# b4rtaz/distributed-llama

Measured on AMD Instinct MI355X. Metric: decode tokens/s (Llama-3.1-8B Q40), higher is better.
Workload: dtype f32-accum/int8-dot (Q40 weights, Q80 activations); 1 GPU; model=llama-3.1-8b, global_batch=1, seq_len=4096, prefill=32, parallelism=tp1, sync=q80, graph=True

## Files before the change

dllama_amd/ops/csrc/gemv.hip:

```cpp

#include "dllama_common.h"

__device__ __forceinline__ int q40_block_dot(const uint4 wq, const int4 x0,
                                             const int4 x1) {
    const uint32_t wv[4] = {wq.x, wq.y, wq.z, wq.w};
    const int32_t xv[8] = {x0.x, x0.y, x0.z, x0.w, x1.x, x1.y, x1.z, x1.w};
    int idot = 0;
    #pragma unroll
    for (int wi = 0; wi < 4; wi++) {
        idot = dot4((int)(wv[wi] & 0x0F0F0F0Fu), xv[wi], idot);
        idot = dot4((int)((wv[wi] >> 4) & 0x0F0F0F0Fu), xv[4 + wi], idot);
    }
    return idot;
}

#define EPI_NONE 0
#define EPI_PACK 4
#define EPI_RESID_Q 3
#define EPI_RESID 1
#define EPI_ROPE 2

template <int NB, int RPW, int EPI, int PRO>
__global__ void k_q40_gemv(const uint8_t *__restrict__ qs,
                           const __half *__restrict__ scales,
                           const int8_t *__restrict__ xq,
                           const float *__restrict__ xs,
                           const float *__restrict__ xbs,
                           float *__restrict__ y,
                           int d, int n,
                           unsigned long long *__restrict__ amax_scratch,
                           float *__restrict__ x_resid,
                           float *__restrict__ ssq,
                           const float *__restrict__ rope_cache,
                           const int *__restrict__ pos,
                           float *__restrict__ kc,
                           float *__restrict__ vc,
                           int q_dim0, int kv_dim0, int hd,
                           const float *__restrict__ wnorm,
                           const float *__restrict__ ssq_in,
                           float eps, int kv_f16,
                           int8_t *__restrict__ oqq,
                           float *__restrict__ oqs,
                           float *__restrict__ oqbs) {
    const int wpb = blockDim.x / WAVE;
    const int wid = threadIdx.x / WAVE;
    const int row0 = (blockIdx.x * wpb + wid) * RPW;
    const int lane = threadIdx.x % WAVE;
    const int nb = n / QB;
    const int nbp = nb >> 1;
    const int nks = gridDim.y;
    const int j0p = (int)((int64_t)nbp * blockIdx.y / nks);
    const int j1p = (int)((int64_t)nbp * (blockIdx.y + 1) / nks);
    const bool wave_valid = row0 < d;
    const int rbase = wave_valid ? row0 : 0;
    [[maybe_unused]] __shared__ float svq[32];

    const uint4 *wrow[RPW];
    const __half *srow[RPW];
    #pragma unroll
    for (int r = 0; r < RPW; r++) {
        const int row = min(rbase + r, d - 1);
        wrow[r] = reinterpret_cast<const uint4 *>(qs + (int64_t)row * (n >> 1));
        srow[r] = scales + (int64_t)row * nb;
    }

    float acc[RPW][NB];
    #pragma unroll
    for (int r = 0; r < RPW; r++)
        #pragma unroll
        for (int b = 0; b < NB; b++) acc[r][b] = 0.0f;

    for (int jp = j0p + lane; jp < j1p; jp += WAVE) {
        const int j = jp << 1;
        uint4 wq0[RPW], wq1[RPW];
        float2 sw[RPW];
        #pragma unroll
        for (int r = 0; r < RPW; r++) {
            wq0[r] = wrow[r][j];
            wq1[r] = wrow[r][j + 1];
            sw[r] = __half22float2(*reinterpret_cast<const __half2 *>(srow[r] + j));
        }
        #pragma unroll
        for (int b = 0; b < NB; b++) {
            const int4 *xrow = reinterpret_cast<const int4 *>(xq + (int64_t)b * n) + j * 2;
            const int4 x0 = xrow[0], x1 = xrow[1], x2 = xrow[2], x3 = xrow[3];
            const float2 sx = *reinterpret_cast<const float2 *>(xs + (int64_t)b * nb + j);
            const float2 bsum = *reinterpret_cast<const float2 *>(xbs + (int64_t)b * nb + j);
            #pragma unroll
            for (int r = 0; r < RPW; r++) {
                const int idot0 = q40_block_dot(wq0[r], x0, x1);
                const int idot1 = q40_block_dot(wq1[r], x2, x3);
                acc[r][b] = fmaf(sw[r].x * sx.x, (float)idot0 - 8.0f * bsum.x, acc[r][b]);
                acc[r][b] = fmaf(sw[r].y * sx.y, (float)idot1 - 8.0f * bsum.y, acc[r][b]);
            }
        }
    }
    if ((nb & 1) && lane == 0 && blockIdx.y == nks - 1) {
        const int j = nb - 1;
        #pragma unroll
        for (int r = 0; r < RPW; r++) {
            const uint4 wq = wrow[r][j];
            const float sw1 = __half2float(srow[r][j]);
            #pragma unroll
            for (int b = 0; b < NB; b++) {
                const int4 *xb = reinterpret_cast<const int4 *>(xq + (int64_t)b * n) + j * 2;
                const float sx1 = xs[(int64_t)b * nb + j];
                const float bs1 = xbs[(int64_t)b * nb + j];
                const int idot = q40_block_dot(wq, xb[0], xb[1]);
                acc[r][b] = fmaf(sw1 * sx1, (float)idot - 8.0f * bs1, acc[r][b]);
            }
        }
    }

    unsigned long long wave_best = 0ull;
    float ssq_local[NB];
    #pragma unroll
    for (int b = 0; b < NB; b++) ssq_local[b] = 0.0f;
    const int pos0 = (EPI == EPI_ROPE) ? pos[0] : 0;

    #pragma unroll
    for (int b = 0; b < NB; b++) {
        float v[RPW];
        float inv = 1.0f;
        if (PRO == 2)
            inv = rsqrtf(ssq_total_wave(ssq_in, b, lane) / n + eps);
        #pragma unroll
        for (int r = 0; r < RPW; r++) {
            v[r] = wave_reduce_sum(acc[r][b]);
            if (PRO == 2) v[r] *= inv;
        }
        if (lane != 0 || !wave_valid) continue;
        if (EPI == EPI_ROPE) {
            const int pb = pos0 + b;
            if (rbase < q_dim0) {
                const int j = (rbase % hd) >> 1;
                const float cr = rope_cache[(int64_t)pb * hd + 2 * j];
                const float ci = rope_cache[(int64_t)pb * hd + 2 * j + 1];
                y[(int64_t)b * d + rbase] = v[0] * cr - v[1 % RPW] * ci;
                y[(int64_t)b * d + rbase + 1] = v[0] * ci + v[1 % RPW] * cr;
            } else if (rbase < q_dim0 + kv_dim0) {
                const int rk = rbase - q_dim0;
                const int j = (rk % hd) >> 1;
                const float cr = rope_cache[(int64_t)pb * hd + 2 * j];
                const float ci = rope_cache[(int64_t)pb * hd + 2 * j + 1];
                const float o0 = v[0] * cr - v[1 % RPW] * ci;
                const float o1 = v[0] * ci + v[1 % RPW] * cr;
                if (kv_f16) {
                    __half *kh = reinterpret_cast<__half *>(kc);
                    kh[(int64_t)pb * kv_dim0 + rk] = __float2half(o0);
                    kh[(int64_t)pb * kv_dim0 + rk + 1] = __float2half(o1);
                } else {
                    kc[(int64_t)pb * kv_dim0 + rk] = o0;
                    kc[(int64_t)pb * kv_dim0 + rk + 1] = o1;
                }
            } else {
                const int rv = rbase - q_dim0 - kv_dim0;
                if (kv_f16) {
                    __half *vh = reinterpret_cast<__half *>(vc);
                    vh[(int64_t)pb * kv_dim0 + rv] = __float2half(v[0]);
                    if (RPW == 2)
                        vh[(int64_t)pb * kv_dim0 + rv + 1] = __float2half(v[1 % RPW]);
                } else {
                    vc[(int64_t)pb * kv_dim0 + rv] = v[0];
                    if (RPW == 2) vc[(int64_t)pb * kv_dim0 + rv + 1] = v[1 % RPW];
                }
            }
        } else {
            #pragma unroll
            for (int r = 0; r < RPW; r++) {
                const int row = rbase + r;
                if (row >= d) continue;
                if (EPI == EPI_RESID) {
                    const float xv = x_resid[(int64_t)b * d + row] + v[r];
                    x_resid[(int64_t)b * d + row] = xv;
                    ssq_local[b] += xv * xv;
                } else if (EPI == EPI_RESID_Q) {
                    const float xv = x_resid[(int64_t)b * d + row] + v[r];
                    x_resid[(int64_t)b * d + row] = xv;
                    ssq_local[b] += xv * xv;
                    svq[wid * RPW + r] = xv * wnorm[row];
                } else if (EPI == EPI_PACK) {
                    svq[wid * RPW + r] = v[r];
                } else {
                    y[((int64_t)b + (int64_t)blockIdx.y * NB) * d + row] = v[r];
                    if (NB == 1) wave_best = max(wave_best, argmax_pack(v[r], row));
                }
            }
        }
    }
    if (EPI == EPI_NONE && NB == 1 && amax_scratch != nullptr) {
        __shared__ unsigned long long wb[16];
        if (lane == 0) wb[wid] = wave_best;
        __syncthreads();
        if (threadIdx.x == 0) {
            unsigned long long best = wb[0];
            for (int i = 1; i < wpb; i++) best = max(best, wb[i]);
            amax_scratch[blockIdx.x] = best;
        }
    }
    if constexpr (EPI == EPI_PACK) {
        __syncthreads();
        if (threadIdx.x < 32 && (int)(blockIdx.x * 32 + threadIdx.x) < d) {
            const Q80Lane c = q80_quant_group32(svq[threadIdx.x]);
            uint8_t *buf = reinterpret_cast<uint8_t *>(oqq);
            buf[blockIdx.x * QB + threadIdx.x] = (uint8_t)(int8_t)c.qf;
            if (threadIdx.x == 0) wire_store_scale(buf, d, blockIdx.x, c.d);
        }
    }
    if constexpr (EPI == EPI_RESID_Q) {
        __shared__ float sredq[16];
        if (lane == 0) sredq[wid] = wave_valid ? ssq_local[0] : 0.0f;
        __syncthreads();
        if (threadIdx.x == 0) {
            float t = 0.0f;
            for (int wv = 0; wv < wpb; wv++) t += sredq[wv];
            atomicAdd(ssq_slot(ssq, 0, blockIdx.x), t);
        }
        if (threadIdx.x < 32 && (int)(blockIdx.x * 32 + threadIdx.x) < d) {
            const Q80Lane c = q80_quant_group32(svq[threadIdx.x]);
            oqq[blockIdx.x * QB + threadIdx.x] = (int8_t)c.qf;
            const float bsq = group32_reduce_sum(c.qf);
            if (threadIdx.x == 0) {
                oqs[blockIdx.x] = c.d;
                oqbs[blockIdx.x] = bsq;
            }
        }
    }
    if (EPI == EPI_RESID) {
        __shared__ float sred[4][NB];
        if (lane == 0)
            #pragma unroll
            for (int b = 0; b < NB; b++) sred[wid][b] = wave_valid ? ssq_local[b] : 0.0f;
        __syncthreads();
        if (threadIdx.x < NB) {
            float t = 0.0f;
            for (int wv = 0; wv < wpb; wv++) t += sred[wv][threadIdx.x];
            atomicAdd(ssq_slot(ssq, threadIdx.x, blockIdx.x), t);
        }
    }
}

template <int LPP, bool GATE = false>
__global__ void k_q40_gemv_grouped(const uint8_t *__restrict__ qs,
                                   const __half *__restrict__ scales,
                                   const int8_t *__restrict__ xq,
                                   const float *__restrict__ xs,
                                   const float *__restrict__ xbs,
                                   const int *__restrict__ expert_idx,
                                   float *__restrict__ y,
                                   int d, int n, int k_slots,
                                   const float *__restrict__ router,
                                   int n_experts, int topk,
                                   const float *__restrict__ ssq_in,
                                   float eps) {
    constexpr int NGRP = WAVE / LPP;
    const int wpb = blockDim.x / WAVE;
    const int full_lane = threadIdx.x % WAVE;
    const int grp = full_lane / LPP;
    const int row0 = ((blockIdx.x * wpb + threadIdx.x / WAVE) * NGRP + grp) * 2;
    const int slot = blockIdx.y;
    if (row0 >= d) return;
    const int lane = full_lane % LPP;
    const int nb = n / QB;
    const int nbp = nb >> 1;
    int e;
    if constexpr (GATE) {
        int gi[16];
        float gw[16];
        const int br = slot / topk, want = slot - br * topk;
        moe_gate_wave(router + (int64_t)br * n_experts, n_experts, topk,
                      full_lane, gi, gw);
        e = 0;
        #pragma unroll
        for (int t = 0; t < 16; t++)
            if (t == want) e = gi[t];
    } else {
        e = expert_idx[slot];
    }
    const int b = slot / k_slots;
    const int row1 = min(row0 + 1, d - 1);
    const uint4 *wrow0 = reinterpret_cast<const uint4 *>(
        qs + ((int64_t)e * d + row0) * (n >> 1));
    const uint4 *wrow1 = reinterpret_cast<const uint4 *>(
        qs + ((int64_t)e * d + row1) * (n >> 1));
    const __half *srow0 = scales + ((int64_t)e * d + row0) * nb;
    const __half *srow1 = scales + ((int64_t)e * d + row1) * nb;
    float acc0 = 0.0f, acc1 = 0.0f;
    for (int jp = lane; jp < nbp; jp += LPP) {
        const int j = jp << 1;
        const uint4 a0 = wrow0[j], a1 = wrow0[j + 1];
        const uint4 b0 = wrow1[j], b1 = wrow1[j + 1];
        const float2 sw0 = __half22float2(*reinterpret_cast<const __half2 *>(srow0 + j));
        const float2 sw1 = __half22float2(*reinterpret_cast<const __half2 *>(srow1 + j));
        const int4 *xr = reinterpret_cast<const int4 *>(xq + (int64_t)b * n) + j * 2;
        const int4 x0 = xr[0], x1 = xr[1], x2 = xr[2], x3 = xr[3];
        const float2 sx = *reinterpret_cast<const float2 *>(xs + (int64_t)b * nb + j);
        const float2 bsum = *reinterpret_cast<const float2 *>(xbs + (int64_t)b * nb + j);
        acc0 = fmaf(sw0.x * sx.x, (float)q40_block_dot(a0, x0, x1) - 8.0f * bsum.x, acc0);
        acc0 = fmaf(sw0.y * sx.y, (float)q40_block_dot(a1, x2, x3) - 8.0f * bsum.y, acc0);
        acc1 = fmaf(sw1.x * sx.x, (float)q40_block_dot(b0, x0, x1) - 8.0f * bsum.x, acc1);
        acc1 = fmaf(sw1.y * sx.y, (float)q40_block_dot(b1, x2, x3) - 8.0f * bsum.y, acc1);
    }
    if ((nb & 1) && lane == 0) {
        const int j = nb - 1;
        const int4 *xb = reinterpret_cast<const int4 *>(xq + (int64_t)b * n) + j * 2;
        acc0 = fmaf(__half2float(srow0[j]) * xs[(int64_t)b * nb + j],
                    (float)q40_block_dot(wrow0[j], xb[0], xb[1])
                    - 8.0f * xbs[(int64_t)b * nb + j], acc0);
        acc1 = fmaf(__half2float(srow1[j]) * xs[(int64_t)b * nb + j],
                    (float)q40_block_dot(wrow1[j], xb[0], xb[1])
                    - 8.0f * xbs[(int64_t)b * nb + j], acc1);
    }
    #pragma unroll
    for (int o = LPP / 2; o > 0; o >>= 1) {
        acc0 += __shfl_down(acc0, o, WAVE);
        acc1 += __shfl_down(acc1, o, WAVE);
    }
    if (ssq_in != nullptr) {
        const float inv = rsqrtf(
            ssq_total_wave(ssq_in, b, threadIdx.x % WAVE) / n + eps);
        acc0 *= inv;
        acc1 *= inv;
    }
    if (lane == 0) {
        y[(int64_t)slot * d + row0] = acc0;
        if (row0 + 1 < d) y[(int64_t)slot * d + row0 + 1] = acc1;
    }
}

template <bool GELU>
__global__ __launch_bounds__(1024) void k_q40_gemv_swiglu(
        const uint8_t *__restrict__ qs, const __half *__restrict__ scales,
        const int8_t *__restrict__ xq, const float *__restrict__ xs,
        const float *__restrict__ xbs, int ff, int n,
        int8_t *__restrict__ oq, float *__restrict__ os,
        float *__restrict__ obs) {
    const int wave = threadIdx.x / WAVE;
    const int lane = threadIdx.x % WAVE;
    const int i0 = blockIdx.x * 32 + 2 * wave;
    const int nb = n / QB, nbp = nb >> 1;
    const int rows[4] = {i0, i0 + 1, ff + i0, ff + i0 + 1};
    const uint4 *wrow[4];
    const __half *srow[4];
    #pragma unroll
    for (int r = 0; r < 4; r++) {
        wrow[r] = reinterpret_cast<const uint4 *>(qs + (int64_t)rows[r] * (n >> 1));
        srow[r] = scales + (int64_t)rows[r] * nb;
    }
    float acc[4] = {0.0f, 0.0f, 0.0f, 0.0f};
    for (int jp = lane; jp < nbp; jp += WAVE) {
        const int j = jp << 1;
        const int4 *xr = reinterpret_cast<const int4 *>(xq) + j * 2;
        const int4 x0 = xr[0], x1 = xr[1], x2 = xr[2], x3 = xr[3];
        const float2 sx = *reinterpret_cast<const float2 *>(xs + j);
        const float2 bsum = *reinterpret_cast<const float2 *>(xbs + j);
        #pragma unroll
        for (int r = 0; r < 4; r++) {
            const uint4 w0 = wrow[r][j], w1 = wrow[r][j + 1];
            const float2 sw = __half22float2(*reinterpret_cast<const __half2 *>(srow[r] + j));
            acc[r] = fmaf(sw.x * sx.x, (float)q40_block_dot(w0, x0, x1) - 8.0f * bsum.x, acc[r]);
            acc[r] = fmaf(sw.y * sx.y, (float)q40_block_dot(w1, x2, x3) - 8.0f * bsum.y, acc[r]);
        }
    }
    if ((nb & 1) && lane == 0) {
        const int j = nb - 1;
        const int4 *xb = reinterpret_cast<const int4 *>(xq) + j * 2;
        const float sx1 = xs[j], bs1 = xbs[j];
        #pragma unroll
        for (int r = 0; r < 4; r++)
            acc[r] = fmaf(__half2float(srow[r][j]) * sx1,
                          (float)q40_block_dot(wrow[r][j], xb[0], xb[1]) - 8.0f * bs1,
                          acc[r]);
    }
    #pragma unroll
    for (int r = 0; r < 4; r++) acc[r] = wave_reduce_sum(acc[r]);
    __shared__ float sv[32];
    if (lane == 0) {
        #pragma unroll
        for (int t = 0; t < 2; t++) {
            const float av = acc[t], gv = acc[2 + t];
            const float act = GELU
                ? 0.5f * av * (1.0f + tanhf(0.797884560802865f * (av + 0.044715f * av * av * av)))
                : av / (1.0f + __expf(-av));
            sv[2 * wave + t] = act * gv;
        }
    }
    __syncthreads();
    if (threadIdx.x < 32) {
        const Q80Lane c = q80_quant_group32(sv[threadIdx.x]);
        oq[(int64_t)blockIdx.x * QB + threadIdx.x] = (int8_t)c.qf;
        const float bsum = group32_reduce_sum(c.qf);
        if (threadIdx.x == 0) { os[blockIdx.x] = c.d; obs[blockIdx.x] = bsum; }
    }
}

template <bool GELU>
__global__ __launch_bounds__(1024) void k_q40_gemv_grouped_swiglu(
        const uint8_t *__restrict__ qs, const __half *__restrict__ scales,
        const int8_t *__restrict__ xq, const float *__restrict__ xs,
        const float *__restrict__ xbs, int ff, int n,
        const float *__restrict__ router, int n_experts, int topk,
        int8_t *__restrict__ oq, float *__restrict__ os,
        float *__restrict__ obs) {
    const int wave = threadIdx.x / WAVE;
    const int lane = threadIdx.x % WAVE;
    const int slot = blockIdx.y;
    const int br = slot / topk, want = slot - br * topk;
    int gi[16];
    float gw[16];
    moe_gate_wave(router + (int64_t)br * n_experts, n_experts, topk, lane, gi, gw);
    int e = 0;
    #pragma unroll
    for (int t = 0; t < 16; t++)
        if (t == want) e = gi[t];
    const int i0 = blockIdx.x * 32 + 2 * wave;
    const int nb = n / QB, nbp = nb >> 1;
    const int rows[4] = {i0, i0 + 1, ff + i0, ff + i0 + 1};
    const uint4 *wrow[4];
    const __half *srow[4];
    #pragma unroll
    for (int r = 0; r < 4; r++) {
        const int64_t rbase = (int64_t)e * 2 * ff + rows[r];
        wrow[r] = reinterpret_cast<const uint4 *>(qs + rbase * (n >> 1));
        srow[r] = scales + rbase * nb;
    }
    const int8_t *xrow = xq + (int64_t)br * n;
    const float *xsr = xs + (int64_t)br * nb;
    const float *xbr = xbs + (int64_t)br * nb;
    float acc[4] = {0.0f, 0.0f, 0.0f, 0.0f};
    for (int jp = lane; jp < nbp; jp += WAVE) {
        const int j = jp << 1;
        const int4 *xr = reinterpret_cast<const int4 *>(xrow) + j * 2;
        const int4 x0 = xr[0], x1 = xr[1], x2 = xr[2], x3 = xr[3];
        const float2 sx = *reinterpret_cast<const float2 *>(xsr + j);
        const float2 bsum = *reinterpret_cast<const float2 *>(xbr + j);
        #pragma unroll
        for (int r = 0; r < 4; r++) {
            const uint4 w0 = wrow[r][j], w1 = wrow[r][j + 1];
            const float2 sw = __half22float2(*reinterpret_cast<const __half2 *>(srow[r] + j));
            acc[r] = fmaf(sw.x * sx.x, (float)q40_block_dot(w0, x0, x1) - 8.0f * bsum.x, acc[r]);
            acc[r] = fmaf(sw.y * sx.y, (float)q40_block_dot(w1, x2, x3) - 8.0f * bsum.y, acc[r]);
        }
    }
    if ((nb & 1) && lane == 0) {
        const int j = nb - 1;
        const int4 *xb = reinterpret_cast<const int4 *>(xrow) + j * 2;
        const float sx1 = xsr[j], bs1 = xbr[j];
        #pragma unroll
        for (int r = 0; r < 4; r++)
            acc[r] = fmaf(__half2float(srow[r][j]) * sx1,
                          (float)q40_block_dot(wrow[r][j], xb[0], xb[1]) - 8.0f * bs1,
                          acc[r]);
    }
    #pragma unroll
    for (int r = 0; r < 4; r++) acc[r] = wave_reduce_sum(acc[r]);
    __shared__ float sv[32];
    if (lane == 0) {
        #pragma unroll
        for (int t = 0; t < 2; t++) {
            const float av = acc[t], gv = acc[2 + t];
            const float act = GELU
                ? 0.5f * av * (1.0f + tanhf(0.797884560802865f * (av + 0.044715f * av * av * av)))
                : av / (1.0f + __expf(-av));
            sv[2 * wave + t] = act * gv;
        }
    }
    __syncthreads();
    if (threadIdx.x < 32) {
        const Q80Lane c = q80_quant_group32(sv[threadIdx.x]);
        oq[((int64_t)slot * ff) + blockIdx.x * QB + threadIdx.x] = (int8_t)c.qf;
        const float bsum = group32_reduce_sum(c.qf);
        if (threadIdx.x == 0) {
            os[(int64_t)slot * (ff / QB) + blockIdx.x] = c.d;
            obs[(int64_t)slot * (ff / QB) + blockIdx.x] = bsum;
        }
    }
}

__global__ void k_add_ssq_q(float *__restrict__ x,
                            const float *__restrict__ parts,
                            float *__restrict__ ssq,
                            const float *__restrict__ wnorm,
                            int8_t *__restrict__ oq,
                            float *__restrict__ os,
                            float *__restrict__ obs,
                            int n, int nks) {
    const int i = blockIdx.x * 256 + threadIdx.x;
    float acc = x[i];
    for (int k = 0; k < nks; k++)
        acc += parts[(int64_t)k * n + i];
    x[i] = acc;
    ssq_block_add<4>(ssq, 0, acc * acc);
    const Q80Lane c = q80_quant_group32(acc * wnorm[i]);
    oq[i] = (int8_t)c.qf;
    const float bsum = group32_reduce_sum(c.qf);
    if ((threadIdx.x & 31) == 0) {
        os[i / QB] = c.d;
        obs[i / QB] = bsum;
    }
}


struct GemvEpi {
    unsigned long long *slot = nullptr;
    float *x_resid = nullptr;
    float *ssq = nullptr;
    const float *cache = nullptr;
    const int *pos = nullptr;
    float *kc = nullptr;
    float *vc = nullptr;
    int q_dim0 = 0, kv_dim0 = 0, hd = 0;
    int kv_f16 = 0;
    bool force_rpw2 = false;
    int ksplit = 1;
    const float *ssq_in = nullptr;
    float eps = 0.0f;
    const float *wnorm = nullptr;
    int8_t *oqq = nullptr;
    float *oqs = nullptr;
    float *oqbs = nullptr;
};

static int gemv_rpw1(int64_t d, bool force_rpw2) {
    static const int rpw1_max =
        std::getenv("DLLAMA_RPW1_MAX") ? atoi(std::getenv("DLLAMA_RPW1_MAX")) : 0;
    return (force_rpw2 || (d >= 2048 && d > rpw1_max)) ? 2 : 1;
}

template <int EPI, int PRO>
static void gemv_launch(torch::Tensor &qs, torch::Tensor &scales, torch::Tensor &xq,
                        torch::Tensor &xs, torch::Tensor &xbs, float *y,
                        int64_t batch, const GemvEpi &e) {
    const int d = qs.size(0);
    const int n = qs.size(1) * 2;
    TORCH_CHECK(xq.size(-1) == n, "x width mismatch");
    TORCH_CHECK(n % QB == 0, "n must be a multiple of 32");
    const int waves_per_block = (EPI == EPI_RESID_Q || EPI == EPI_PACK) ? 16 : 4;
    const dim3 block(waves_per_block * WAVE);
    auto launch = [&](auto nb_const, auto rpw_const) {
        constexpr int RPW = decltype(rpw_const)::value;
        const dim3 grid(ceil_div(d, waves_per_block * RPW), e.ksplit);
        hipLaunchKernelGGL((k_q40_gemv<decltype(nb_const)::value, RPW, EPI, PRO>), grid,
                           block, 0, cur_stream(),
                           qs.data_ptr<uint8_t>(),
                           reinterpret_cast<const __half *>(scales.data_ptr<at::Half>()),
                           xq.data_ptr<int8_t>(), xs.data_ptr<float>(),
                           xbs.data_ptr<float>(), y, d, n,
                           e.slot, e.x_resid, e.ssq,
                           e.cache, e.pos, e.kc, e.vc, e.q_dim0, e.kv_dim0, e.hd,
                           e.wnorm, e.ssq_in, e.eps, e.kv_f16,
                           e.oqq, e.oqs, e.oqbs);
    };
    std::integral_constant<int, 1> r1;
    std::integral_constant<int, 2> r2;
    auto launch_nb = [&](auto nb_const) {
        constexpr int NB = decltype(nb_const)::value;
        if constexpr (EPI == EPI_ROPE || NB == 2 || NB == 4) {
            launch(nb_const, r2);
        } else if constexpr (NB > 4) {
            launch(nb_const, r1);
        } else {
            if (gemv_rpw1(d, e.force_rpw2) == 2) launch(nb_const, r2);
            else launch(nb_const, r1);
        }
    };
    switch (batch) {
        case 1: launch_nb(std::integral_constant<int, 1>{}); break;
        case 2: launch_nb(std::integral_constant<int, 2>{}); break;
        case 4: launch_nb(std::integral_constant<int, 4>{}); break;
        case 8:
        case 16:
        case 32:
            if constexpr (PRO) {
                TORCH_CHECK(false, "fused-norm GEMV supports batch <= 4");
            } else {
                if (batch == 8) launch_nb(std::integral_constant<int, 8>{});
                else if (batch == 16) launch_nb(std::integral_constant<int, 16>{});
                else launch_nb(std::integral_constant<int, 32>{});
            }
            break;
        default: TORCH_CHECK(false, "unsupported batch ", batch);
    }
}

void q40_gemv(torch::Tensor qs, torch::Tensor scales, torch::Tensor xq,
              torch::Tensor xs, torch::Tensor xbs, torch::Tensor y, int64_t batch,
              c10::optional<torch::Tensor> amax_slot = c10::nullopt,
              c10::optional<torch::Tensor> ssq_in = c10::nullopt,
              double eps = 0.0) {
    CHECK_CUDA(qs); CHECK_CONT(qs); CHECK_CONT(xq);
    GemvEpi e;
    if (amax_slot.has_value())
        e.slot = reinterpret_cast<unsigned long long *>(amax_slot->data_ptr<int64_t>());
    if (ssq_in.has_value()) {
        e.ssq_in = ssq_in->data_ptr<float>();
        e.eps = (float)eps;
        gemv_launch<EPI_NONE, 2>(qs, scales, xq, xs, xbs, y.data_ptr<float>(), batch, e);
    } else {
        gemv_launch<EPI_NONE, 0>(qs, scales, xq, xs, xbs, y.data_ptr<float>(), batch, e);
    }
}

void q40_gemv_pack(torch::Tensor qs, torch::Tensor scales, torch::Tensor xq,
                   torch::Tensor xs, torch::Tensor xbs, torch::Tensor wire) {
    CHECK_CUDA(qs); CHECK_CONT(qs); CHECK_CONT(xq);
    const int d = qs.size(0);
    TORCH_CHECK(d % 32 == 0, "gemv_pack needs d % 32 == 0");
    GemvEpi e;
    e.oqq = reinterpret_cast<int8_t *>(wire.data_ptr<uint8_t>());
    e.force_rpw2 = true;
    gemv_launch<EPI_PACK, 0>(qs, scales, xq, xs, xbs, nullptr, 1, e);
}

void q40_gemv_ksplit(torch::Tensor qs, torch::Tensor scales, torch::Tensor xq,
                     torch::Tensor xs, torch::Tensor xbs, torch::Tensor part,
                     int64_t ks) {
    CHECK_CUDA(qs); CHECK_CONT(qs); CHECK_CONT(xq);
    TORCH_CHECK((int64_t)ks * qs.size(0) <= part.numel(), "part buffer too small");
    GemvEpi e;
    e.force_rpw2 = true;
    e.ksplit = (int)ks;
    gemv_launch<EPI_NONE, 0>(qs, scales, xq, xs, xbs, part.data_ptr<float>(), 1, e);
}

void add_ssq_q(torch::Tensor x, torch::Tensor parts, torch::Tensor ssq,
               torch::Tensor wnorm, torch::Tensor oq, torch::Tensor os,
               torch::Tensor obs, int64_t nks) {
    CHECK_CUDA(x);
    const int n = x.size(-1);
    TORCH_CHECK(n % 256 == 0, "add_ssq_q needs dim % 256 == 0");
    hipLaunchKernelGGL(k_add_ssq_q, dim3(n / 256), dim3(256), 0, cur_stream(),
                       x.data_ptr<float>(), parts.data_ptr<float>(),
                       ssq.data_ptr<float>(), wnorm.data_ptr<float>(),
                       oq.data_ptr<int8_t>(), os.data_ptr<float>(),
                       obs.data_ptr<float>(), n, (int)nks);
}

void q40_gemv_resid_q(torch::Tensor qs, torch::Tensor scales, torch::Tensor xq,
                      torch::Tensor xs, torch::Tensor xbs, torch::Tensor x,
                      torch::Tensor ssq, torch::Tensor wnorm, torch::Tensor oq,
                      torch::Tensor os, torch::Tensor obs) {
    CHECK_CUDA(qs); CHECK_CONT(qs); CHECK_CONT(xq);
    const int d = qs.size(0);
    TORCH_CHECK(d % 32 == 0, "resid_q needs d % 32 == 0");
    GemvEpi e;
    e.x_resid = x.data_ptr<float>();
    e.ssq = ssq.data_ptr<float>();
    e.wnorm = wnorm.data_ptr<float>();
    e.oqq = oq.data_ptr<int8_t>();
    e.oqs = os.data_ptr<float>();
    e.oqbs = obs.data_ptr<float>();
    e.force_rpw2 = true;
    gemv_launch<EPI_RESID_Q, 0>(qs, scales, xq, xs, xbs, x.data_ptr<float>(), 1, e);
}

void q40_gemv_resid(torch::Tensor qs, torch::Tensor scales, torch::Tensor xq,
                    torch::Tensor xs, torch::Tensor xbs, torch::Tensor x,
                    torch::Tensor ssq, int64_t batch) {
    CHECK_CUDA(qs); CHECK_CONT(qs); CHECK_CONT(xq);
    TORCH_CHECK(batch <= 32, "RESID epilogue LDS sized for batch<=32");
    GemvEpi e;
    e.x_resid = x.data_ptr<float>();
    e.ssq = ssq.data_ptr<float>();
    gemv_launch<EPI_RESID, 0>(qs, scales, xq, xs, xbs, x.data_ptr<float>(), batch, e);
}

void q40_gemv_rope(torch::Tensor qs, torch::Tensor scales, torch::Tensor xq,
                   torch::Tensor xs, torch::Tensor xbs, torch::Tensor y,
                   int64_t batch, torch::Tensor cache, torch::Tensor pos,
                   torch::Tensor kc, torch::Tensor vc, int64_t q_dim0,
                   int64_t kv_dim0, int64_t head_dim,
                   c10::optional<torch::Tensor> ssq_in = c10::nullopt,
                   double eps = 0.0) {
    CHECK_CUDA(qs); CHECK_CONT(qs); CHECK_CONT(xq);
    GemvEpi e;
    e.cache = cache.data_ptr<float>();
    e.pos = pos.data_ptr<int>();
    e.kv_f16 = kc.scalar_type() == at::kHalf ? 1 : 0;
    e.kc = static_cast<float *>(kc.data_ptr());
    e.vc = static_cast<float *>(vc.data_ptr());
    e.q_dim0 = (int)q_dim0;
    e.kv_dim0 = (int)kv_dim0;
    e.hd = (int)head_dim;
    e.force_rpw2 = true;
    if (ssq_in.has_value()) {
        e.ssq_in = ssq_in->data_ptr<float>();
        e.eps = (float)eps;
        gemv_launch<EPI_ROPE, 2>(qs, scales, xq, xs, xbs, y.data_ptr<float>(), batch, e);
    } else {
        gemv_launch<EPI_ROPE, 0>(qs, scales, xq, xs, xbs, y.data_ptr<float>(), batch, e);
    }
}

int64_t q40_gemv_argmax_blocks(int64_t d) {
    return ceil_div(d, 4 * gemv_rpw1(d, false));
}

void q40_gemv_grouped(torch::Tensor qs, torch::Tensor scales, torch::Tensor xq,
                      torch::Tensor xs, torch::Tensor xbs, torch::Tensor expert_idx,
                      torch::Tensor y, int64_t k_slots, int64_t variant = -1,
                      c10::optional<torch::Tensor> router = c10::nullopt,
                      int64_t topk = 0, int64_t n_slots_override = 0,
                      c10::optional<torch::Tensor> ssq_in = c10::nullopt,
                      double eps = 0.0) {
    CHECK_CUDA(qs); CHECK_CONT(qs);
    const int d = qs.size(1);
    const int n = qs.size(2) * 2;
    const int n_slots = n_slots_override > 0 ? (int)n_slots_override
                                             : (int)expert_idx.numel();
    const int waves_per_block = 4;
    static const bool env_v2 = !std::getenv("DLLAMA_MOE_V2")
        || atoi(std::getenv("DLLAMA_MOE_V2")) != 0;
    int lpp = 64;
    if (variant < 0 ? env_v2 : variant == 1) {
        const int nbp = (n / QB) >> 1;
        lpp = 8;
        while (lpp < nbp && lpp < 64) lpp <<= 1;
    }
    const int rows_per_wg = waves_per_block * 2 * (WAVE / lpp);
    const dim3 grid(ceil_div(d, rows_per_wg), n_slots);
    const dim3 block(waves_per_block * WAVE);
    const bool gate = router.has_value();
    const float *rp = gate ? router->data_ptr<float>() : nullptr;
    const int ne = gate ? (int)router->size(-1) : 0;
    const float *sqp = ssq_in.has_value() ? ssq_in->data_ptr<float>() : nullptr;
    auto launch = [&](auto k) {
        hipLaunchKernelGGL(k, grid, block, 0, cur_stream(),
                           qs.data_ptr<uint8_t>(),
                           reinterpret_cast<const __half *>(scales.data_ptr<at::Half>()),
                           xq.data_ptr<int8_t>(), xs.data_ptr<float>(),
                           xbs.data_ptr<float>(), expert_idx.data_ptr<int>(),
                           y.data_ptr<float>(), d, n, (int)k_slots,
                           rp, ne, (int)topk, sqp, (float)eps);
    };
    if (gate) {
        switch (lpp) {
            case 8: launch(k_q40_gemv_grouped<8, true>); break;
            case 16: launch(k_q40_gemv_grouped<16, true>); break;
            case 32: launch(k_q40_gemv_grouped<32, true>); break;
            default: launch(k_q40_gemv_grouped<64, true>); break;
        }
    } else {
        switch (lpp) {
            case 8: launch(k_q40_gemv_grouped<8>); break;
            case 16: launch(k_q40_gemv_grouped<16>); break;
            case 32: launch(k_q40_gemv_grouped<32>); break;
            default: launch(k_q40_gemv_grouped<64>); break;
        }
    }
}

void q40_gemv_swiglu(torch::Tensor qs, torch::Tensor scales, torch::Tensor xq,
                     torch::Tensor xs, torch::Tensor xbs, torch::Tensor oq,
                     torch::Tensor os, torch::Tensor obs, bool gelu = false) {
    CHECK_CUDA(qs); CHECK_CONT(qs); CHECK_CONT(xq);
    const int d = qs.size(0);
    const int ff = d / 2;
    const int n = qs.size(1) * 2;
    TORCH_CHECK(ff % 32 == 0, "fused swiglu GEMV needs ff % 32 == 0");
    TORCH_CHECK(xq.size(-1) == n, "x width mismatch");
    const dim3 grid(ff / 32);
    const dim3 block(16 * WAVE);
    auto launch = [&](auto k) {
        hipLaunchKernelGGL(k, grid, block, 0, cur_stream(),
                           qs.data_ptr<uint8_t>(),
                           reinterpret_cast<const __half *>(scales.data_ptr<at::Half>()),
                           xq.data_ptr<int8_t>(), xs.data_ptr<float>(),
                           xbs.data_ptr<float>(), ff, n,
                           oq.data_ptr<int8_t>(), os.data_ptr<float>(),
                           obs.data_ptr<float>());
    };
    if (gelu) launch(k_q40_gemv_swiglu<true>);
    else launch(k_q40_gemv_swiglu<false>);
}

void q40_gemv_grouped_swiglu(torch::Tensor qs, torch::Tensor scales,
                             torch::Tensor xq, torch::Tensor xs,
                             torch::Tensor xbs, torch::Tensor oq,
                             torch::Tensor os, torch::Tensor obs,
                             int64_t n_slots, torch::Tensor router,
                             int64_t topk, bool gelu = false) {
    CHECK_CUDA(qs); CHECK_CONT(qs); CHECK_CONT(xq);
    const int ff = (int)qs.size(1) / 2;
    const int n = (int)qs.size(2) * 2;
    TORCH_CHECK(ff % 32 == 0, "fused grouped swiglu needs ff % 32 == 0");
    const dim3 grid(ff / 32, n_slots);
    const dim3 block(16 * WAVE);
    auto launch = [&](auto k) {
        hipLaunchKernelGGL(k, grid, block, 0, cur_stream(),
                           qs.data_ptr<uint8_t>(),
                           reinterpret_cast<const __half *>(scales.data_ptr<at::Half>()),
                           xq.data_ptr<int8_t>(), xs.data_ptr<float>(),
                           xbs.data_ptr<float>(), ff, n,
                           router.data_ptr<float>(), (int)router.size(-1),
                           (int)topk, oq.data_ptr<int8_t>(),
                           os.data_ptr<float>(), obs.data_ptr<float>());
    };
    if (gelu) launch(k_q40_gemv_grouped_swiglu<true>);
    else launch(k_q40_gemv_grouped_swiglu<false>);
}

void register_gemv(py::module &m) {
    m.def("q40_gemv", &q40_gemv, py::arg("qs"), py::arg("scales"), py::arg("xq"),
          py::arg("xs"), py::arg("xbs"), py::arg("y"), py::arg("batch"),
          py::arg("amax_slot") = py::none(), py::arg("ssq_in") = py::none(),
          py::arg("eps") = 0.0);
    m.def("q40_gemv_resid", &q40_gemv_resid);
    m.def("q40_gemv_resid_q", &q40_gemv_resid_q);
    m.def("q40_gemv_pack", &q40_gemv_pack);
    m.def("q40_gemv_ksplit", &q40_gemv_ksplit);
    m.def("add_ssq_q", &add_ssq_q);
    m.def("q40_gemv_rope", &q40_gemv_rope, py::arg("qs"), py::arg("scales"),
          py::arg("xq"), py::arg("xs"), py::arg("xbs"), py::arg("y"),
          py::arg("batch"), py::arg("cache"), py::arg("pos"), py::arg("kc"),
          py::arg("vc"), py::arg("q_dim0"), py::arg("kv_dim0"),
          py::arg("head_dim"), py::arg("ssq_in") = py::none(),
          py::arg("eps") = 0.0);
    m.def("q40_gemv_swiglu", &q40_gemv_swiglu, py::arg("qs"), py::arg("scales"),
          py::arg("xq"), py::arg("xs"), py::arg("xbs"), py::arg("oq"),
          py::arg("os"), py::arg("obs"), py::arg("gelu") = false);
    m.def("q40_gemv_grouped", &q40_gemv_grouped, py::arg("qs"),
          py::arg("scales"), py::arg("xq"), py::arg("xs"), py::arg("xbs"),
          py::arg("expert_idx"), py::arg("y"), py::arg("k_slots"),
          py::arg("variant") = -1, py::arg("router") = py::none(),
          py::arg("topk") = 0, py::arg("n_slots") = 0,
          py::arg("ssq_in") = py::none(), py::arg("eps") = 0.0);
    m.def("q40_gemv_grouped_swiglu", &q40_gemv_grouped_swiglu, py::arg("qs"),
          py::arg("scales"), py::arg("xq"), py::arg("xs"), py::arg("xbs"),
          py::arg("oq"), py::arg("os"), py::arg("obs"), py::arg("n_slots"),
          py::arg("router"), py::arg("topk"), py::arg("gelu") = false);
    m.def("q40_gemv_argmax_blocks", &q40_gemv_argmax_blocks);
}
```

Before: 575.0 tokens/s.

## Split resid_q gemv blocks with last-block ticket hand-off for Q80 quantization

Adds an EPI_RESID_QH variant of the residual+quantize GEMV epilogue that runs with fewer waves per block (8 by default for narrow-output, wide-input matrices). Each 32-row quantization group is then spread across several blocks. Blocks write their residual pairs atomically, take a per-group ticket, and the last arriving block re-reads the group and produces the Q80 output. The aim is more blocks in flight and better latency hiding on the down projection, at the cost of extra atomics, a per-buffer ticket allocation, and a requirement to run once eagerly before graph capture.

```diff
diff --git a/dllama_amd/ops/csrc/gemv.hip b/dllama_amd/ops/csrc/gemv.hip
--- a/dllama_amd/ops/csrc/gemv.hip
+++ b/dllama_amd/ops/csrc/gemv.hip
@@ -1,5 +1,10 @@
 
 #include "dllama_common.h"
+
+#include <atomic>
+#include <mutex>
+#include <unordered_map>
+#include <vector>
 
 __device__ __forceinline__ int q40_block_dot(const uint4 wq, const int4 x0,
                                              const int4 x1) {
@@ -17,6 +22,7 @@
 #define EPI_NONE 0
 #define EPI_PACK 4
 #define EPI_RESID_Q 3
+#define EPI_RESID_QH 5
 #define EPI_RESID 1
 #define EPI_ROPE 2
 
@@ -69,6 +75,18 @@
     for (int r = 0; r < RPW; r++)
         #pragma unroll
         for (int b = 0; b < NB; b++) acc[r][b] = 0.0f;
+
+    static_assert(EPI != EPI_RESID_QH || (RPW == 2 && NB == 1),
+                  "the hand-off epilogue is B=1, RPW=2");
+    [[maybe_unused]] float xres[2] = {0.0f, 0.0f};
+    if constexpr (EPI == EPI_RESID_QH) {
+        if (lane == 0) {
+            #pragma unroll
+            for (int r = 0; r < 2; r++)
+                xres[r] = __hip_atomic_load(&x_resid[rbase + r], __ATOMIC_RELAXED,
+                                            __HIP_MEMORY_SCOPE_WAVEFRONT);
+        }
+    }
 
     for (int jp = j0p + lane; jp < j1p; jp += WAVE) {
         const int j = jp << 1;
@@ -165,6 +183,15 @@
                     if (RPW == 2) vc[(int64_t)pb * kv_dim0 + rv + 1] = v[1 % RPW];
                 }
             }
+        } else if constexpr (EPI == EPI_RESID_QH) {
+            const float xv0 = xres[0] + v[0];
+            const float xv1 = xres[1] + v[1 % RPW];
+            ssq_local[b] += xv0 * xv0;
+            ssq_local[b] += xv1 * xv1;
+            const unsigned long long pk = (unsigned long long)__float_as_uint(xv0)
+                | ((unsigned long long)__float_as_uint(xv1) << 32);
+            __hip_atomic_store(reinterpret_cast<unsigned long long *>(x_resid + rbase),
+                               pk, __ATOMIC_RELAXED, __HIP_MEMORY_SCOPE_AGENT);
         } else {
             #pragma unroll
             for (int r = 0; r < RPW; r++) {
@@ -223,6 +250,43 @@
             if (threadIdx.x == 0) {
                 oqs[blockIdx.x] = c.d;
                 oqbs[blockIdx.x] = bsq;
+            }
+        }
+    }
+    if constexpr (EPI == EPI_RESID_QH) {
+        asm volatile("s_waitcnt vmcnt(0)" ::: "memory");
+        __shared__ float sredq[8];
+        __shared__ unsigned slast;
+        if (lane == 0) sredq[wid] = wave_valid ? ssq_local[0] : 0.0f;
+        __syncthreads();
+        unsigned *tickets = reinterpret_cast<unsigned *>(amax_scratch);
+        const unsigned per = 16u / (unsigned)wpb;
+        const unsigned blk = blockIdx.x / per;
+        if (threadIdx.x == 0) {
+            float t = 0.0f;
+            for (int wv = 0; wv < wpb; wv++) t += sredq[wv];
+            const unsigned prev = __hip_atomic_fetch_add(
+                tickets + blk, 1u, __ATOMIC_RELAXED, __HIP_MEMORY_SCOPE_AGENT);
+            atomicAdd(ssq_slot(ssq, 0, blockIdx.x), t);
+            const unsigned last = prev == per - 1u;
+            if (last)
+                __hip_atomic_store(tickets + blk, 0u, __ATOMIC_RELAXED,
+                                   __HIP_MEMORY_SCOPE_AGENT);
+            slast = last;
+        }
+        __syncthreads();
+        if (!slast) return;
+        __builtin_amdgcn_fence(__ATOMIC_ACQUIRE, "wavefront");
+        if (threadIdx.x < 32 && (int)(blk * 32 + threadIdx.x) < d) {
+            const int row = blk * 32 + threadIdx.x;
+            const float xv = __hip_atomic_load(&x_resid[row], __ATOMIC_RELAXED,
+                                               __HIP_MEMORY_SCOPE_AGENT);
+            const Q80Lane c = q80_quant_group32(xv * wnorm[row]);
+            oqq[blk * QB + threadIdx.x] = (int8_t)c.qf;
+            const float bsq = group32_reduce_sum(c.qf);
+            if (threadIdx.x == 0) {
+                oqs[blk] = c.d;
+                oqbs[blk] = bsq;
             }
         }
     }
@@ -519,6 +583,7 @@
     int8_t *oqq = nullptr;
     float *oqs = nullptr;
     float *oqbs = nullptr;
+    int waves = 0;
 };
 
 static int gemv_rpw1(int64_t d, bool force_rpw2) {
@@ -535,7 +600,8 @@
     const int n = qs.size(1) * 2;
     TORCH_CHECK(xq.size(-1) == n, "x width mismatch");
     TORCH_CHECK(n % QB == 0, "n must be a multiple of 32");
-    const int waves_per_block = (EPI == EPI_RESID_Q || EPI == EPI_PACK) ? 16 : 4;
+    const int waves_per_block = (EPI == EPI_RESID_QH) ? e.waves
+        : (EPI == EPI_RESID_Q || EPI == EPI_PACK) ? 16 : 4;
     const dim3 block(waves_per_block * WAVE);
     auto launch = [&](auto nb_const, auto rpw_const) {
         constexpr int RPW = decltype(rpw_const)::value;
@@ -555,7 +621,10 @@
     std::integral_constant<int, 2> r2;
     auto launch_nb = [&](auto nb_const) {
         constexpr int NB = decltype(nb_const)::value;
-        if constexpr (EPI == EPI_ROPE || NB == 2 || NB == 4) {
+        if constexpr (EPI == EPI_RESID_QH) {
+            if constexpr (NB == 1) launch(nb_const, r2);
+            else TORCH_CHECK(false, "resid_q hand-off form is batch 1 only");
+        } else if constexpr (EPI == EPI_ROPE || NB == 2 || NB == 4) {
             launch(nb_const, r2);
         } else if constexpr (NB > 4) {
             launch(nb_const, r1);
@@ -636,6 +705,49 @@
                        obs.data_ptr<float>(), n, (int)nks);
 }
 
+static std::atomic<int> g_resid_q_waves_override{0};
+
+static int resid_q_waves(int d, int n) {
+    static const int env_waves =
+        std::getenv("DLLAMA_RESID_Q_WAVES") ? atoi(std::getenv("DLLAMA_RESID_Q_WAVES")) : 0;
+    const int ov = g_resid_q_waves_override.load();
+    const int forced = ov ? ov : env_waves;
+    if (forced == 4 || forced == 8 || forced == 16) return forced;
+    return (d < 8192 && n >= 8192) ? 8 : 16;
+}
+
+void q40_gemv_resid_q_waves(int64_t waves) {
+    TORCH_CHECK(waves == 0 || waves == 4 || waves == 8 || waves == 16,
+                "resid_q waves: 0 (default rule), 4, 8 or 16");
+    g_resid_q_waves_override.store((int)waves);
+}
+
+static unsigned *resid_q_tickets(const torch::Tensor &x, int nblocks) {
+    static std::mutex mu;
+    static auto *store = new std::unordered_map<const void *, torch::Tensor>();
+    static auto *outgrown = new std::vector<torch::Tensor>();
+    std::lock_guard<std::mutex> lock(mu);
+    const void *key = x.data_ptr();
+    auto it = store->find(key);
+    if (it != store->end() && it->second.numel() >= nblocks)
+        return reinterpret_cast<unsigned *>(it->second.data_ptr<int32_t>());
+    hipStreamCaptureStatus st = hipStreamCaptureStatusNone;
+    C10_HIP_CHECK(hipStreamIsCapturing(cur_stream(), &st));
+    TORCH_CHECK(st == hipStreamCaptureStatusNone,
+                "q40_gemv_resid_q: first use of this residual buffer (or with "
+                "a larger d) inside stream capture; run the call eagerly once "
+                "before capturing so its block tickets exist");
+    torch::Tensor t = torch::zeros({nblocks}, x.options().dtype(torch::kInt32));
+    C10_HIP_CHECK(hipStreamSynchronize(cur_stream()));
+    if (it != store->end()) {
+        outgrown->push_back(it->second);
+        it->second = t;
+    } else {
+        store->emplace(key, t);
+    }
+    return reinterpret_cast<unsigned *>(t.data_ptr<int32_t>());
+}
+
 void q40_gemv_resid_q(torch::Tensor qs, torch::Tensor scales, torch::Tensor xq,
                       torch::Tensor xs, torch::Tensor xbs, torch::Tensor x,
                       torch::Tensor ssq, torch::Tensor wnorm, torch::Tensor oq,
@@ -643,6 +755,10 @@
     CHECK_CUDA(qs); CHECK_CONT(qs); CHECK_CONT(xq);
     const int d = qs.size(0);
     TORCH_CHECK(d % 32 == 0, "resid_q needs d % 32 == 0");
+    TORCH_CHECK(x.numel() >= d && wnorm.numel() >= d && oq.numel() >= d,
+                "resid_q: x, wnorm and oq need d elements");
+    TORCH_CHECK(reinterpret_cast<uintptr_t>(x.data_ptr<float>()) % 8 == 0,
+                "resid_q: x must be 8-byte aligned (row pairs are stored whole)");
     GemvEpi e;
     e.x_resid = x.data_ptr<float>();
     e.ssq = ssq.data_ptr<float>();
@@ -651,7 +767,14 @@
     e.oqs = os.data_ptr<float>();
     e.oqbs = obs.data_ptr<float>();
     e.force_rpw2 = true;
-    gemv_launch<EPI_RESID_Q, 0>(qs, scales, xq, xs, xbs, x.data_ptr<float>(), 1, e);
+    const int waves = resid_q_waves(d, (int)qs.size(1) * 2);
+    if (waves == 16) {
+        gemv_launch<EPI_RESID_Q, 0>(qs, scales, xq, xs, xbs, x.data_ptr<float>(), 1, e);
+    } else {
+        e.waves = waves;
+        e.slot = reinterpret_cast<unsigned long long *>(resid_q_tickets(x, d / 32));
+        gemv_launch<EPI_RESID_QH, 0>(qs, scales, xq, xs, xbs, x.data_ptr<float>(), 1, e);
+    }
 }
 
 void q40_gemv_resid(torch::Tensor qs, torch::Tensor scales, torch::Tensor xq,
@@ -807,6 +930,7 @@
           py::arg("eps") = 0.0);
     m.def("q40_gemv_resid", &q40_gemv_resid);
     m.def("q40_gemv_resid_q", &q40_gemv_resid_q);
+    m.def("q40_gemv_resid_q_waves", &q40_gemv_resid_q_waves);
     m.def("q40_gemv_pack", &q40_gemv_pack);
     m.def("q40_gemv_ksplit", &q40_gemv_ksplit);
     m.def("add_ssq_q", &add_ssq_q);
```

New measurement: 605.4 tokens/s (median of 6 runs). 1.05x the previous value.
